# fakerlove1/HPFG

Hardware: AMD Instinct MI355X
Metric: labeled+unlabeled images/sec/node, U-Net 224x224 ACDC-shaped (Mean-Teacher step) (higher is better)
Workload: dtype bf16x3 (fp32 storage; products as split-bf16 MFMA hi*hi+hi*lo+lo*hi, fp32 accumulate); 1 GPU; mean_teacher_unet_224x224 (BASELINE configs[1]): U-Net 1ch->4cls, 8 labelled + 8 unlabelled per GPU, student fwd+bwd + train-mode teacher fwd + CE/Dice/MSE + SGD + EMA; size=224, hipgraph=True, sync_bn=False, parallelism=dp1, math=bf16x3

## Files before the change

hpfg_amd/_lib.py:

```python
from __future__ import annotations

import ctypes as C
import os
import threading

_HERE = os.path.dirname(os.path.abspath(__file__))
LIB_PATH = os.path.join(_HERE, "lib", "libhpfg_hip.so")

BN_MEAN, BN_RSTD, BN_SCALE, BN_SHIFT, BN_K1, BN_K2, BN_K3, BN_SPARE, BN_ROWS = range(9)
ACT_NONE, ACT_PLAIN, ACT_STRIDED, ACT_BNACT, ACT_BNACT_POOL, ACT_UP2X, ACT_DZ, ACT_SPLIT16, ACT_UPBWD = range(9)
OPT_CONV_THIN, OPT_FIRST_MFMA, OPT_FIRST_WGRAD, OPT_NARROW_DEEP, OPT_UPDATE_PACK = 0, 1, 2, 3, 4
LOSS_NSUM = 32
LOSS_MAX_CLASSES = 16
ACC_MAX_SHARDS = 8
VERSION = 141
RESIZE_TAPS = 36
SURFACE_SEGS = 32
MATH_F32, MATH_BF16X3 = 0, 1


class HipLibraryError(RuntimeError):
    pass


class Act(C.Structure):
    _fields_ = [("z", C.c_void_p), ("bn", C.c_void_p), ("aux", C.c_void_p), ("mode", C.c_int32), ("C", C.c_int32),
                ("Hs", C.c_int32), ("Ws", C.c_int32), ("pstride", C.c_int32), ("aux_pstride", C.c_int32),
                ("bn_stride", C.c_int32), ("bn_coff", C.c_int32), ("sn", C.c_int32), ("sc", C.c_int32), ("sy", C.c_int32),
                ("sx", C.c_int32), ("drop_p", C.c_float), ("drop_seed", C.c_uint32), ("drop_mask", C.c_void_p), ("seed_dev", C.c_void_p),
                ("bn_acc", C.c_void_p), ("bn_gamma", C.c_void_p), ("bn_beta", C.c_void_p), ("bn_count", C.c_float), ("bn_eps", C.c_float),
                ("bn_shards", C.c_int32), ("reserved1", C.c_int32)]


class ConvArgs(C.Structure):
    _fields_ = [("a0", Act), ("a1", Act), ("wpk", C.c_void_p), ("bias", C.c_void_p), ("out", C.c_void_p),
                ("stat_partials", C.c_void_p), ("out_pstride", C.c_int32), ("Cout", C.c_int32), ("CoutPad", C.c_int32),
                ("N", C.c_int32), ("H", C.c_int32), ("W", C.c_int32), ("taps", C.c_int32), ("math", C.c_int32),
                ("bwd_stats", C.c_int32), ("bwd_of", Act), ("out2", C.c_void_p), ("out_split", C.c_int32), ("out2_pstride", C.c_int32),
                ("stat_acc", C.c_void_p), ("stat_shards", C.c_int32), ("reserved2", C.c_int32), ("stage_out", C.c_void_p), ("side_sums", C.c_void_p)]


class WgradArgs(C.Structure):
    _fields_ = [("a0", Act), ("a1", Act), ("g", Act), ("slab", C.c_void_p), ("dw_oihw", C.c_void_p), ("Cin", C.c_int32),
                ("CinPad", C.c_int32), ("Cout", C.c_int32), ("CoutPad", C.c_int32), ("N", C.c_int32), ("H", C.c_int32),
                ("W", C.c_int32), ("taps", C.c_int32), ("S", C.c_int32), ("math", C.c_int32), ("defer_reduce", C.c_int32)]


class PeerX(C.Structure):
    _fields_ = [("mbox", C.c_void_p * 8), ("epoch", C.c_void_p), ("err", C.c_void_p), ("world", C.c_int32), ("rank", C.c_int32),
                ("slot", C.c_int32), ("cap", C.c_int32), ("slot_bytes", C.c_int64)]


class PeerBuf(C.Structure):
    _fields_ = [("win", C.c_void_p * 8), ("epoch", C.c_void_p), ("err", C.c_void_p), ("world", C.c_int32), ("rank", C.c_int32),
                ("slice", C.c_int64), ("n", C.c_int64), ("stride", C.c_int64)]


class FusedBwdArgs(C.Structure):
    _fields_ = [("d", ConvArgs), ("xa0", Act), ("xa1", Act), ("slab", C.c_void_p), ("Cin", C.c_int32), ("CinPad", C.c_int32),
                ("Cout", C.c_int32), ("CoutPad", C.c_int32)]


class AugSample(C.Structure):
    _fields_ = [("img_off", C.c_int64), ("lab_off", C.c_int64), ("h", C.c_int32), ("w", C.c_int32), ("mode", C.c_int32), ("k", C.c_int32),
# ... 162 lines not shown
    "hpfg_gelu_bwd": (_i, [_p, _p, _p, _l, _p]),
    "hpfg_patch_merge_fwd": (_i, [_p, _p, _i, _i, _i, _i, _p]),
    "hpfg_patch_merge_bwd": (_i, [_p, _p, _i, _i, _i, _i, _p]),
    "hpfg_attn_fwd_hd": (_i, [_p, _p, _p, _i, _i, _i, _i, _i, _f, _p]),
    "hpfg_attn_bwd_hd": (_i, [_p, _p, _p, _p, _p, _p, _i, _i, _i, _i, _i, _f, _p]),
    "hpfg_gemm_f32": (_i, [_p, _l, _l, _p, _l, _l, _p, _l, _i, _i, _i, _p, _i, _i, _p]),
    "hpfg_gemm_f32_splitk": (_i, [_p, _l, _l, _p, _l, _l, _p, _l, _i, _i, _i, _p, _i, _i, _p, _p]),
    "hpfg_gemm_f32_splits": (_i, [_i, _i, _i]),
    "hpfg_gemm_bf16x3": (_i, [_p, _l, _l, _p, _l, _l, _p, _l, _i, _i, _i, _p, _i, _i, _p]),
    "hpfg_gemm_bf16x3_splits": (_i, [_i, _i, _i]),
    "hpfg_gemm_bf16x3_splitk": (_i, [_p, _l, _l, _p, _l, _l, _p, _l, _i, _i, _i, _p, _i, _i, _p, _p]),
    "hpfg_gemm_bf16x3_ok": (_i, [_p, _l, _l, _p, _l, _l, _i, _i, _i]),
    "hpfg_gemm_tn_bf16x3": (_i, [_p, _p, _p, _p, _l, _i, _i, _i, _p]),
    "hpfg_gemm_tn_splits": (_i, [_l, _i, _i]),
    "hpfg_col_sum2": (_i, [_p, _l, _i, _l, _p, _p, _p]),
    "hpfg_col_sum_splits": (_i, [_l]),
    "hpfg_col_sum": (_i, [_p, _l, _i, _l, _p, _p]),
    "hpfg_relu_bwd": (_i, [_p, _p, _l, _p]),
    "hpfg_neck_pool_fwd": (_i, [_p, _i, _i, _i, _i, _i, _i, _p, _p, _p]),
    "hpfg_neck_pool_bwd": (_i, [_p, _p, _i, _i, _i, _i, _i, _p, _p]),
    "hpfg_l2norm_fwd": (_i, [_p, _i, _i, _i, _i, _i, _p, _p, _p]),
    "hpfg_l2norm_bwd": (_i, [_p, _p, _p, _i, _i, _i, _i, _i, _p, _p, _p]),
    "hpfg_ntxent_rows": (_i, [_p, _i, _f, _p, _p, _p]),
}

_lock = threading.Lock()
_lib = None


def load() -> C.CDLL:
    global _lib
    if _lib is not None:
        return _lib
    with _lock:
        if _lib is not None:
            return _lib
        if not os.path.exists(LIB_PATH):
            raise HipLibraryError(
                f"{LIB_PATH} not found: build it with `python -c 'import __graft_entry__ as g; g.build()'` "
                f"or `make -C hpfg_amd/csrc`. There is no CPU fallback for the HIP path.")
        lib = C.CDLL(LIB_PATH)
        for name, (res, args) in PROTOTYPES.items():
            fn = getattr(lib, name)
            fn.restype = res
            fn.argtypes = args
        if lib.hpfg_version() != VERSION:
            raise HipLibraryError(f"libhpfg_hip.so version {lib.hpfg_version()} != binding version {VERSION}; rebuild")
        if os.environ.get("HPFG_FIRST_WGRAD", "1") == "0":
            lib.hpfg_set_option(OPT_FIRST_WGRAD, 0)
        if os.environ.get("HPFG_NARROW_DEEP") is not None:
            lib.hpfg_set_option(OPT_NARROW_DEEP, int(os.environ["HPFG_NARROW_DEEP"]))
        if os.environ.get("HPFG_UPDATE_PACK", "1") == "0":
            lib.hpfg_set_option(OPT_UPDATE_PACK, 0)
        _lib = lib
    return _lib


def check(rc: int, what: str):
    if rc != 0:
        msg = load().hpfg_last_error().decode("utf-8", "replace")
        raise HipLibraryError(f"{what} failed (rc={rc}): {msg}")


def ptr(t):
    return None if t is None else t.data_ptr()


def none_act() -> Act:
    return Act()
```

hpfg_amd/csrc/conv_bf16_kernel.h:

```cpp
#pragma once
#include <stdlib.h>
#include "stage.h"

namespace hpfg_conv16 {

using namespace hpfg_stage;

template <int TH_, int TW_, int WM_, int WN_, int NI_, int TAPS_, int KC_>
struct Cfg {
  static constexpr int TH = TH_, TW = TW_, WM = WM_, WN = WN_, NI = NI_, TAPS = TAPS_, KC = KC_;
  static constexpr int MI = TH * TW / 16 / WM;
  static constexpr int BN = 16 * NI * WN;
  static constexpr int HALO = TAPS == 9 ? 1 : 0;
  static constexpr int HP = TH + 2 * HALO, WP = TW + 2 * HALO;
  static constexpr int RS = TW == 16 ? WP : (TAPS == 9 ? 24 : 8);
  static constexpr int NSLOT = (HP * RS + 15) / 16 * 16;
  static constexpr int NG = KC / 8;
  static constexpr int PLANE = NSLOT * 16;
  static constexpr int BUF_BYTES = NG * 2 * PLANE;
  static constexpr int KSTEPS = TAPS == 1 ? 1 : (KC == 32 ? 9 : 5);
  static constexpr int NPIECE = HP * WP * NG;
  static constexpr int NLD = (NPIECE + 255) / 256;
  static_assert(WM * WN == 4, "4 waves per workgroup");
  static_assert(256 % NG == 0, "a thread must keep one channel group");
  static_assert(KC == 32 || (KC == 16 && TAPS == 9), "two-tap K packing only for 3x3");
  static_assert(TAPS == 1 || NLD + 2 <= KSTEPS, "stage pipeline must fit into the k-steps of a chunk");
};

struct Piece {
  int ly, lx, lds, ok;
};
template <class C>
__device__ __forceinline__ Piece make_piece(int tid, int i) {
  Piece q;
  const int idx = tid + i * 256;
  const int pix = idx / C::NG, g = idx % C::NG;
  q.ok = idx < C::NPIECE;
  q.ly = pix / C::WP - C::HALO;
  q.lx = pix % C::WP - C::HALO;
  q.lds = (g * 2) * C::PLANE + ((pix / C::WP) * C::RS + pix % C::WP) * 16;
  return q;
}

template <class C, int KIND = HPFG_KIND_PLAIN, bool SIDE_ON = false>
__device__ __forceinline__ void store_piece(unsigned char* buf, const Piece& q, const f32x4& v0, const f32x4& v1, const HpfgConvArgs* p = nullptr,
                                            bool on = false, int n = 0, int gy = 0, int gx = 0, int c0 = 0, bool ok = false) {
  if (!q.ok) return;
  bf16x8 hi, lo;
  split_piece<KIND>(v0, v1, hi, lo);
  *reinterpret_cast<bf16x8*>(buf + q.lds) = hi;
  *reinterpret_cast<bf16x8*>(buf + q.lds + C::PLANE) = lo;
  if constexpr (SIDE_ON) {
    if (on && ok && q.ly >= 0 && q.ly < C::TH && q.lx >= 0 && q.lx < C::TW) {
      const int ct = p->a0.C + p->a1.C;
      __bf16* d = reinterpret_cast<__bf16*>(p->stage_out) + ((((long)n * p->H + gy) * p->W + gx) * ct + c0) * 2;
      *reinterpret_cast<bf16x8*>(d) = hi;
      *reinterpret_cast<bf16x8*>(d + 8) = lo;
    }
  }
}

template <class C>
__device__ __forceinline__ void load_b(bf16x8 (&bh)[C::NI], bf16x8 (&bl)[C::NI], const bf16x8* wpk, int ks, int ntn, int nt0, int lane) {
#pragma unroll
  for (int j = 0; j < C::NI; ++j) {
    const bf16x8* q = wpk + ((ks * ntn + nt0 + j) * 2) * 64 + lane;
    bh[j] = q[0];
    bl[j] = q[64];
  }
}

template <class C>
__device__ __forceinline__ void conv16_load_bias(const HpfgConvArgs& p, f32x4 (&bias)[C::NI], int lane, int nt0) {
#pragma unroll
// ... 135 lines not shown
      }
      s1[j][r] = a;
      s2[j][r] = b;
    }
  if ((lane & 15) == 0) {
#pragma unroll
    for (int j = 0; j < C::NI; ++j) {
      const int cl = (wn * C::NI + j) * 16 + (lane >> 4) * 4;
      *reinterpret_cast<f32x4*>(ldsf + (0 * C::WM + wm) * C::BN + cl) = s1[j];
      *reinterpret_cast<f32x4*>(ldsf + (1 * C::WM + wm) * C::BN + cl) = s2[j];
    }
  }
  __syncthreads();
  if (tid < 2 * C::BN) {
    const int which = tid / C::BN, cl = tid % C::BN;
    float t = 0.f;
#pragma unroll
    for (int w = 0; w < C::WM; ++w) t += ldsf[(which * C::WM + w) * C::BN + cl];
    const int co = cb * C::BN + cl;
    if (BWD && p.bwd_stats && which == 1 && co < p.Cout) {
      float sg = 0.f;
#pragma unroll
      for (int w = 0; w < C::WM; ++w) sg += ldsf[w * C::BN + cl];
      const float* tb = p.bwd_of.bn + p.bwd_of.bn_coff + co;
      t = tb[HPFG_BN_RSTD * p.bwd_of.bn_stride] * (t - tb[HPFG_BN_MEAN * p.bwd_of.bn_stride] * sg);
    }
    if (p.stat_acc && co < p.Cout)
      hpfg_acc_add(p.stat_acc, p.CoutPad, ((int)blockIdx.z * (int)gridDim.y + (int)blockIdx.y) * (int)gridDim.x + (int)blockIdx.x & (p.stat_shards - 1), which, co, t);
    if (p.stat_partials && co < p.CoutPad) p.stat_partials[((long)row * 2 + which) * p.CoutPad + co] = t;
  }
}

#define HPFG16_MFMA3(ACC, AH, AL, BH, BL)                              \
  ACC = __builtin_amdgcn_mfma_f32_16x16x32_bf16(BH, AH, ACC, 0, 0, 0); \
  ACC = __builtin_amdgcn_mfma_f32_16x16x32_bf16(BL, AH, ACC, 0, 0, 0); \
  ACC = __builtin_amdgcn_mfma_f32_16x16x32_bf16(BH, AL, ACC, 0, 0, 0);

template <class C>
struct UpGeo {
  using P = UpPatch<C::TH, C::TW>;
  static constexpr int SW = P::SW;
  static constexpr int NPIECE = P::SH * P::SW * C::NG;
  static constexpr int BYTES = P::SH * P::SW * C::KC * 4;
  static_assert(NPIECE <= 256, "one source piece per thread");
};
template <int KIND>
constexpr int eff_nr() { return KIND == HPFG_KIND_CAT ? 2 : RawCount<KIND>::N; }

template <class C, int KIND>
constexpr int wg_per_cu() {
  return (C::KSTEPS == 5 && C::NI == 1 && RawCount<KIND>::N <= 2) ? 3 : 2;
}

template <class C, int KIND, int BWD = 0>
__global__ __launch_bounds__(256, (wg_per_cu<C, KIND>())) void conv_bf16x3_kernel(HpfgConvArgs p, int tiles_x, int tiles_y) {
  static_assert(C::TAPS == 9, "persistent kernel is the 3x3 path");
  constexpr int STAT_BYTES = 2 * 4 * C::BN * 4;
  constexpr int NR = eff_nr<KIND>();
  constexpr bool CATK = KIND == HPFG_KIND_CAT;
  constexpr int UP_BYTES = CATK ? UpGeo<C>::BYTES : 0;
  __shared__ __attribute__((aligned(16))) unsigned char lds[2 * C::BUF_BYTES + STAT_BYTES + UP_BYTES];
  float* ldsf = reinterpret_cast<float*>(lds + 2 * C::BUF_BYTES);
  float* ldsU = reinterpret_cast<float*>(lds + 2 * C::BUF_BYTES + STAT_BYTES);
  (void)ldsU;
  constexpr bool TABK = tab_in_lds<KIND>();
  __shared__ __attribute__((aligned(16))) float ldsBN[TABK ? tab_rows<KIND>() * HPFG_BN_CMAX : 4];
  (void)ldsBN;
  const int tid = threadIdx.x, lane = tid & 63, wave = tid >> 6;
  const int wm = wave % C::WM, wn = wave / C::WM;
  const int cb = blockIdx.y;
  const int H = p.H, W = p.W;
  const int ntiles = tiles_x * tiles_y, nwork = ntiles * p.N;
  const ActCtx cx0 = make_ctx(p.a0);
  constexpr bool SIDE = KIND != HPFG_KIND_PLAIN && C::TH == 4;
  const bool dzw = SIDE && p.stage_out != nullptr && cb == 0;
  (void)dzw;
#ifdef HPFG_TRACE
  const bool tr_on = (p.math & 0x2000) && tid == 0;
  unsigned long long* tr_buf = reinterpret_cast<unsigned long long*>(p.stat_partials) + 256 * ((long)blockIdx.y * gridDim.x + blockIdx.x);
  int tr_i = 0;
#endif
  HPFG_TR_REAL(11)
  HPFG_TR(1)

  f32x4 acc[C::MI][C::NI];
#pragma unroll
  for (int m = 0; m < C::MI; ++m)
#pragma unroll
    for (int j = 0; j < C::NI; ++j) acc[m][j] = f32x4{0.f, 0.f, 0.f, 0.f};

  const int kg = lane >> 4;
  const int gl = C::KC == 32 ? kg : (kg & 1);
  int aoff[C::MI];
#pragma unroll
  for (int m = 0; m < C::MI; ++m) {
    const int pxl = (wm * C::MI + m) * 16 + (lane & 15);
    aoff[m] = (gl * 2) * C::PLANE + ((pxl / C::TW) * C::RS + (pxl % C::TW)) * 16;
  }
  int toff[C::KSTEPS];
#pragma unroll
  for (int s = 0; s < C::KSTEPS; ++s) {
    int tap = C::KC == 32 ? s : 2 * s + (kg >> 1);
    tap = tap > 8 ? 8 : tap;
    toff[s] = ((tap / 3) * C::RS + (tap % 3)) * 16;
  }
  Piece pc[C::NLD];
#pragma unroll
  for (int i = 0; i < C::NLD; ++i) pc[i] = make_piece<C>(tid, i);
  const int g8 = (tid % C::NG) * 8;

  const int cin_total = p.a0.C + p.a1.C;
  const int nchunks = (cin_total + C::KC - 1) / C::KC;
  const int ntn = p.CoutPad / 16;
  const int nt0 = (cb * C::WN + wn) * C::NI;
  const bf16x8* wpk = reinterpret_cast<const bf16x8*>(p.wpk);

  const TileWalk tw = tile_walk(nwork, gridDim.x >= 8 ? 8 : 1);
  const int wend = tw.wend, G = tw.step;
  int w = tw.w;
  if (w >= wend) {
    if (p.stat_partials && threadIdx.x < 2 * C::BN) {
      const int co = cb * C::BN + (int)threadIdx.x % C::BN;
      if (co < p.CoutPad) p.stat_partials[((long)blockIdx.x * 2 + (int)threadIdx.x / C::BN) * p.CoutPad + co] = 0.f;
    }
    return;
  }
  int n = w / ntiles, tyi = (w % ntiles) / tiles_x, txi = (w % ntiles) % tiles_x;
  int ty0 = tyi * C::TH, tx0 = txi * C::TW;
  const int gn = G / ntiles, gty = (G % ntiles) / tiles_x, gtx = (G % ntiles) % tiles_x;
  f32x4 s1[C::NI], s2[C::NI];
#pragma unroll
  for (int j = 0; j < C::NI; ++j) {
    s1[j] = f32x4{0.f, 0.f, 0.f, 0.f};
    s2[j] = s1[j];
  }
  constexpr bool TIGHT = C::TAPS == 9 && C::KSTEPS == 5 && C::NI >= 2 && eff_nr<KIND>() >= 4;
  f32x4 bias[C::NI];
  if (!TIGHT) conv16_load_bias<C>(p, bias, lane, nt0);
  Tab tab;
  HPFG_TR(2)
  {
    const int c0 = g8;
    const bool chv = c0 < cin_total;
    const int c0c = chv ? c0 : 0;
    RawPiece<KIND> raw0[C::NLD];
#pragma unroll
    for (int i = 0; i < C::NLD; ++i) {
      const int gy = ty0 + pc[i].ly, gx = tx0 + pc[i].lx;
      const bool ok = pc[i].ok && chv && gy >= 0 && gy < H && gx >= 0 && gx < W;
      issue_piece<KIND>(raw0[i], p.a0, p.a1, cx0, n, clampi(gy, 0, H - 1), clampi(gx, 0, W - 1), c0c, ok);
    }
    if constexpr (TABK) {
      fill_tables_lds<KIND>(p.a0, ldsBN, p.a0.C, tid, 256);
      __syncthreads();
      load_tables_lds<KIND>(tab, ldsBN, p.a0, c0c);
    } else {
      load_tables<KIND>(tab, p.a0, c0, chv);
    }
#pragma unroll
    for (int i = 0; i < C::NLD; ++i) {
      const int gy = ty0 + pc[i].ly, gx = tx0 + pc[i].lx;
      const bool ok = pc[i].ok && chv && gy >= 0 && gy < H && gx >= 0 && gx < W;
      f32x4 v0, v1;
      const int gyc = clampi(gy, 0, H - 1), gxc = clampi(gx, 0, W - 1);
      finish_piece<KIND>(v0, v1, raw0[i], tab, p.a0, p.a1, cx0, n, gyc, gxc, c0c, ok);
      store_piece<C, KIND, SIDE>(lds, pc[i], v0, v1, &p, dzw, n, gyc, gxc, c0c, ok);
    }
  }
  constexpr int BR = C::KSTEPS == 5 ? 5 : (C::NI == 1 ? 9 : 3), BD = BR - 1;
  static_assert(C::KSTEPS % BR == 0, "ring size must divide the k-steps of a chunk");
  const int kperiod = nchunks * C::KSTEPS;
  bf16x8 bh[BR][C::NI], bl[BR][C::NI];
#pragma unroll
  for (int d = 0; d < BD; ++d) load_b<C>(bh[d], bl[d], wpk, d % kperiod, ntn, nt0, lane);
  HPFG_TR(3)
  __syncthreads();
  HPFG_TR(4)
  int item = 0;
  while (true) {
    for (int ch = 0; ch < nchunks; ++ch, ++item) {
      const unsigned char* cur = lds + (item & 1) * C::BUF_BYTES;
      unsigned char* nxt = lds + ((item + 1) & 1) * C::BUF_BYTES;
      const bool last_chunk = ch + 1 == nchunks;
      const int w2 = w + G;
      const bool more = !last_chunk || w2 < wend;
      const int nch = last_chunk ? 0 : ch + 1;
      int nn = n, nty = ty0, ntx = tx0;
      if (last_chunk && more) {
        int x2 = txi + gtx, y2 = tyi + gty;
        nn = n + gn;
        if (x2 >= tiles_x) {
          x2 -= tiles_x;
          ++y2;
        }
        if (y2 >= tiles_y) {
          y2 -= tiles_y;
          ++nn;
        }
        nty = y2 * C::TH;
        ntx = x2 * C::TW;
      }
      const int c0n = nch * C::KC + g8;
      const bool chvn = more && c0n < cin_total && !(p.math & 0x400);
      const int c0c = c0n < cin_total ? c0n : 0;
      if constexpr (TABK) load_tables_lds<KIND>(tab, ldsBN, p.a0, c0c);
      else if (!TIGHT || (more && nchunks > 1)) load_tables<KIND>(tab, p.a0, c0c, true);
      constexpr bool DEEP = (NR <= 2 || C::NLD <= 2) && (C::KC != 32 || CATK);
      constexpr int SK = CATK ? HPFG_KIND_BNACT : KIND;
      RawPiece<SK> raw[DEEP ? C::NLD : 2];
      const bool up_next = CATK && nch * C::KC >= p.a0.C;
      f32x4 rawU[2];
      int sy_base = 0, sx_base = 0;
      if (CATK && up_next) {
        sy_base = up_base(nty - 1, p.a1.Hs);
        sx_base = up_base(ntx - 1, p.a1.Ws);
        const int cu = (c0n < cin_total ? c0n : p.a0.C) - p.a0.C;
        up_patch_issue<UpGeo<C>::SW>(rawU, p.a1, nn, sy_base, sx_base, tid / C::NG, cu);
      } else if (DEEP) {
#pragma unroll
        for (int i = 0; i < C::NLD; ++i) {
          const int gy = nty + pc[i].ly, gx = ntx + pc[i].lx;
          const bool ok = pc[i].ok && chvn && gy >= 0 && gy < H && gx >= 0 && gx < W;
          issue_piece<SK>(raw[DEEP ? i : 0], p.a0, p.a1, cx0, nn, clampi(gy, 0, H - 1), clampi(gx, 0, W - 1), c0c, ok);
        }
      }
      HPFG_TR(5)
      constexpr int Q = C::KSTEPS * C::MI;
      constexpr int AD0 = wg_per_cu<C, KIND>() == 3 ? 2 : (C::NI == 1 ? 4 : (TIGHT ? 0 : 2));
      constexpr int AD = AD0 < Q ? AD0 : Q;
      constexpr int AR = AD + 1;
      constexpr bool FENCE = !TIGHT;
      bf16x8 ah[AR], al[AR];
#pragma unroll
      for (int q = 0; q < AD; ++q) {
        ah[q % AR] = *reinterpret_cast<const bf16x8*>(cur + aoff[q % C::MI] + toff[q / C::MI]);
        al[q % AR] = *reinterpret_cast<const bf16x8*>(cur + aoff[q % C::MI] + toff[q / C::MI] + C::PLANE);
      }
      if (FENCE) __builtin_amdgcn_sched_barrier(0x216);
#pragma unroll
      for (int q = 0; q < Q; ++q) {
        const int s = q / C::MI, m = q % C::MI;
        if (q + AD < Q) {
          const int q2 = q + AD;
          ah[q2 % AR] = *reinterpret_cast<const bf16x8*>(cur + aoff[q2 % C::MI] + toff[q2 / C::MI]);
          al[q2 % AR] = *reinterpret_cast<const bf16x8*>(cur + aoff[q2 % C::MI] + toff[q2 / C::MI] + C::PLANE);
        }
        if (m == 0) {
          if (!DEEP) {
            if (s >= 2 && s - 2 < C::NLD) {
              const int i = s - 2 < C::NLD ? s - 2 : 0;
              const int gy = nty + pc[i].ly, gx = ntx + pc[i].lx;
              const bool ok = pc[i].ok && chvn && gy >= 0 && gy < H && gx >= 0 && gx < W;
              f32x4 v0, v1;
              finish_piece<SK>(v0, v1, raw[i & 1], tab, p.a0, p.a1, cx0, nn, clampi(gy, 0, H - 1), clampi(gx, 0, W - 1), c0c, ok);
              store_piece<C, SK, SIDE>(nxt, pc[i], v0, v1, &p, dzw, nn, gy, gx, c0c, ok);
            }
            if (s < C::NLD) {
              const int i = s < C::NLD ? s : 0;
              const int gy = nty + pc[i].ly, gx = ntx + pc[i].lx;
              const bool ok = pc[i].ok && chvn && gy >= 0 && gy < H && gx >= 0 && gx < W;
              issue_piece<SK>(raw[i & 1], p.a0, p.a1, cx0, nn, clampi(gy, 0, H - 1), clampi(gx, 0, W - 1), c0c, ok);
            }
          }
          int ksn = ch * C::KSTEPS + s + BD;
          ksn = ksn >= kperiod ? ksn - kperiod : ksn;
          load_b<C>(bh[(s + BD) % BR], bl[(s + BD) % BR], wpk, ksn, ntn, nt0, lane);
        }
#pragma unroll
        for (int j = 0; j < C::NI; ++j) { HPFG16_MFMA3(acc[m][j], ah[q % AR], al[q % AR], bh[s % BR][j], bl[s % BR][j]) }
        if (FENCE) __builtin_amdgcn_sched_barrier(0x216);
      }
      HPFG_TR(6)
      if (CATK && up_next) {
        using UG = UpGeo<C>;
        if (tid < UG::NPIECE) up_patch_park<C::KC>(ldsU, rawU, tid / C::NG, g8);
        __syncthreads();
#pragma unroll
        for (int i = 0; i < C::NLD; ++i) {
          const int gy = nty + pc[i].ly, gx = ntx + pc[i].lx;
          const bool ok = pc[i].ok && chvn && gy >= 0 && gy < H && gx >= 0 && gx < W;
          f32x4 v0, v1;
          up_blend<C::KC, UG::SW>(v0, v1, ldsU, p.a1, clampi(gy, 0, H - 1), clampi(gx, 0, W - 1), sy_base, sx_base, g8, ok);
          store_piece<C, HPFG_KIND_PLAIN, SIDE>(nxt, pc[i], v0, v1, &p, dzw, nn, gy, gx, c0c, ok);
        }
      } else if (DEEP) {
#pragma unroll
        for (int i = 0; i < C::NLD; ++i) {
          const int gy = nty + pc[i].ly, gx = ntx + pc[i].lx;
          const bool ok = pc[i].ok && chvn && gy >= 0 && gy < H && gx >= 0 && gx < W;
          f32x4 v0, v1;
          finish_piece<SK>(v0, v1, raw[DEEP ? i : 0], tab, p.a0, p.a1, cx0, nn, clampi(gy, 0, H - 1), clampi(gx, 0, W - 1), c0c, ok);
          store_piece<C, SK, SIDE>(nxt, pc[i], v0, v1, &p, dzw, nn, gy, gx, c0c, ok);
        }
      }
      HPFG_TR(7)
      __syncthreads();
      HPFG_TR(8)
    }
    conv16_store_tile<C, BWD>(p, acc, s1, s2, bias, lane, wm, nt0, n, ty0, tx0, TIGHT);
    HPFG_TR(9)
#pragma unroll
    for (int m = 0; m < C::MI; ++m)
#pragma unroll
      for (int j = 0; j < C::NI; ++j) acc[m][j] = f32x4{0.f, 0.f, 0.f, 0.f};
    w += G;
    if (w >= wend) break;
    txi += gtx;
    tyi += gty;
    n += gn;
    if (txi >= tiles_x) {
      txi -= tiles_x;
      ++tyi;
    }
    if (tyi >= tiles_y) {
      tyi -= tiles_y;
      ++n;
    }
    ty0 = tyi * C::TH;
    tx0 = txi * C::TW;
  }
  conv16_flush_stats<C, BWD>(p, s1, s2, ldsf, tid, lane, wm, wn, cb, (int)blockIdx.x);
  HPFG_TR(10)
  HPFG_TR_REAL(12)
}

template <class C, int KIND, int BWD = 0>
__global__ __launch_bounds__(256) void conv1x1_bf16x3_kernel(HpfgConvArgs p, int tiles_x, int tiles_y) {
  static_assert(C::TAPS == 1, "1x1 path");
  constexpr int STAT_BYTES = 2 * 4 * C::BN * 4;
  constexpr int NR = RawCount<KIND>::N;
  __shared__ __attribute__((aligned(16))) unsigned char lds[C::BUF_BYTES + STAT_BYTES];
  float* ldsf = reinterpret_cast<float*>(lds + C::BUF_BYTES);
  constexpr bool TABK = tab_in_lds<KIND>();
  __shared__ __attribute__((aligned(16))) float ldsBN[TABK ? tab_rows<KIND>() * HPFG_BN_CMAX : 4];
  (void)ldsBN;
  constexpr bool UPB = KIND == HPFG_KIND_UPB;
  __shared__ short upI[UPB ? C::TH + C::TW : 1][HPFG_UPB_TAPS];
  __shared__ float upW[UPB ? C::TH + C::TW : 1][HPFG_UPB_TAPS];
  __shared__ __attribute__((aligned(16))) float upS[UPB ? 256 * 8 : 4];
  (void)upI;
  (void)upW;
  (void)upS;
  const int tid = threadIdx.x, lane = tid & 63, wave = tid >> 6;
  const int wm = wave % C::WM, wn = wave / C::WM;
  const int tile = blockIdx.x, n = blockIdx.y, cb = blockIdx.z;
  const int ty0 = (tile / tiles_x) * C::TH, tx0 = (tile % tiles_x) * C::TW;
  const int H = p.H, W = p.W;
  const ActCtx cx0 = make_ctx(p.a0);
  f32x4 acc[C::MI][C::NI];
#pragma unroll
  for (int m = 0; m < C::MI; ++m)
#pragma unroll
// ... 91 lines not shown
      }
      if (side && p.side_sums) {
        *reinterpret_cast<f32x4*>(upS + tid * 8) = cs0;
        *reinterpret_cast<f32x4*>(upS + tid * 8 + 4) = cs1;
      }
    } else {
#pragma unroll
    for (int i = 0; i < C::NLD; ++i) {
      const Piece q = make_piece<C>(tid, i);
      const int gy = ty0 + q.ly, gx = tx0 + q.lx;
      const bool ok = q.ok && chv && gy < H && gx < W;
      RawPiece<KIND> raw;
      f32x4 v0, v1;
      const int gyc = clampi(gy, 0, H - 1), gxc = clampi(gx, 0, W - 1), c0c = chv ? c0 : 0;
      issue_piece<KIND>(raw, p.a0, p.a1, cx0, n, gyc, gxc, c0c, ok);
      finish_piece<KIND>(v0, v1, raw, tab, p.a0, p.a1, cx0, n, gyc, gxc, c0c, ok);
      store_piece<C, KIND>(lds, q, v0, v1);
    }
    }
    bf16x8 bh[C::NI], bl[C::NI];
    load_b<C>(bh, bl, wpk, ch, ntn, nt0, lane);
    __syncthreads();
    if constexpr (UPB) {
      if (side && p.side_sums && tid < C::KC) {
        const int g = tid >> 3, j = tid & 7;
        float tsum = 0.f;
        for (int k = g; k < 256; k += C::NG) tsum += upS[k * 8 + j];
        const int cch = ch * C::KC + tid;
        if (cch < p.a0.C) p.side_sums[(long)wg_row * p.a0.C + cch] = tsum;
      }
    }
#pragma unroll
    for (int m = 0; m < C::MI; ++m) {
      const bf16x8 ah = *reinterpret_cast<const bf16x8*>(lds + aoff[m]);
      const bf16x8 al = *reinterpret_cast<const bf16x8*>(lds + aoff[m] + C::PLANE);
#pragma unroll
      for (int j = 0; j < C::NI; ++j) { HPFG16_MFMA3(acc[m][j], ah, al, bh[j], bl[j]) }
    }
  }
  f32x4 s1[C::NI], s2[C::NI];
#pragma unroll
  for (int j = 0; j < C::NI; ++j) {
    s1[j] = f32x4{0.f, 0.f, 0.f, 0.f};
    s2[j] = s1[j];
  }
  f32x4 bias[C::NI];
  conv16_load_bias<C>(p, bias, lane, nt0);
  conv16_store_tile<C, BWD>(p, acc, s1, s2, bias, lane, wm, nt0, n, ty0, tx0);
  __syncthreads();
  conv16_flush_stats<C, BWD>(p, s1, s2, ldsf, tid, lane, wm, wn, cb, n * (tiles_x * tiles_y) + tile);
}

template <class C, int KIND>
int persistent_grid(const HpfgConvArgs& a) {
  const int tx = (a.W + C::TW - 1) / C::TW, ty = (a.H + C::TH - 1) / C::TH;
  const int lds_bytes = 2 * C::BUF_BYTES + 2 * 4 * C::BN * 4;
  int per_cu = 160 * 1024 / lds_bytes;
  const int reg_cap = wg_per_cu<C, KIND>();
  if (per_cu > reg_cap) per_cu = reg_cap;
  if (per_cu < 1) per_cu = 1;
  const long nwork = (long)tx * ty * a.N;
  const long gy = a.CoutPad / C::BN;
  long cap = 256L * per_cu / (gy > 0 ? gy : 1);
  if (cap < 1) cap = 1;
  const long rounds = (nwork + cap - 1) / cap;
  return (int)((nwork + rounds - 1) / rounds);
}

template <class C, int KIND>
int launch_cfg(const HpfgConvArgs& a, hipStream_t st, int* rows_only) {
  int tx = (a.W + C::TW - 1) / C::TW, ty = (a.H + C::TH - 1) / C::TH;
  if (rows_only) {
    if constexpr (C::TAPS == 9) *rows_only = persistent_grid<C, KIND>(a);
    else *rows_only = tx * ty * a.N;
    return 0;
  }
  if constexpr (C::TAPS == 9) {
    dim3 grid((unsigned)persistent_grid<C, KIND>(a), a.CoutPad / C::BN);
    if (a.stat_acc) HPFG_ACC_CHECK((long)grid.x * grid.y, a.stat_shards, "conv_fwd");
    if constexpr (KIND == HPFG_KIND_DZ || KIND == HPFG_KIND_PLAIN) {
      if constexpr (C::TH == 4) {
        if (a.bwd_stats == 2) {
          hipLaunchKernelGGL((conv_bf16x3_kernel<C, KIND, 2>), grid, dim3(256), 0, st, a, tx, ty);
          return hpfg_launch_status("conv_bf16x3_kernel<bwd stats + pool>");
        }
      }
      if (a.bwd_stats == 2) {
        hpfg_set_error("conv_fwd: bwd_stats == 2 is built for H or W not a multiple of 16");
        return -1;
      }
      if (a.bwd_stats) {
        hipLaunchKernelGGL((conv_bf16x3_kernel<C, KIND, 1>), grid, dim3(256), 0, st, a, tx, ty);
        return hpfg_launch_status("conv_bf16x3_kernel<bwd stats>");
      }
    }
    hipLaunchKernelGGL((conv_bf16x3_kernel<C, KIND>), grid, dim3(256), 0, st, a, tx, ty);
  } else {
    dim3 grid(tx * ty, a.N, a.CoutPad / C::BN);
    if (a.stat_acc) HPFG_ACC_CHECK((long)grid.x * grid.y * grid.z, a.stat_shards, "conv_fwd(1x1)");
    if constexpr (KIND == HPFG_KIND_DZ || KIND == HPFG_KIND_PLAIN || KIND == HPFG_KIND_UPB) {
      if (a.bwd_stats) {
        hipLaunchKernelGGL((conv1x1_bf16x3_kernel<C, KIND, 1>), grid, dim3(256), 0, st, a, tx, ty);
        return hpfg_launch_status("conv1x1_bf16x3_kernel<bwd stats>");
      }
    }
    hipLaunchKernelGGL((conv1x1_bf16x3_kernel<C, KIND>), grid, dim3(256), 0, st, a, tx, ty);
  }
  return hpfg_launch_status("conv_bf16x3_kernel");
}

template <int KIND, int TAPS>
int conv_dispatch_kind(const HpfgConvArgs& a, hipStream_t st, int* rows_only) {
  const bool big = (a.H % 16 == 0) && (a.W % 16 == 0);
  const int cp = a.CoutPad;
  constexpr int KCB = TAPS == 9 ? 16 : 32;
  if (big) {
    if constexpr (TAPS == 1) {
      if (cp % 64 == 0) return launch_cfg<Cfg<16, 16, 4, 1, 4, TAPS, KCB>, KIND>(a, st, rows_only);
    }
    if (cp % 32 == 0) return launch_cfg<Cfg<16, 16, 4, 1, 2, TAPS, KCB>, KIND>(a, st, rows_only);
    return launch_cfg<Cfg<16, 16, 4, 1, 1, TAPS, KCB>, KIND>(a, st, rows_only);
  }
  if constexpr (TAPS == 9) {
    {
      const long tiles = (long)a.N * ((a.H + 3) / 4) * ((a.W + 15) / 16);
      if (cp % 64 == 0 && tiles * (cp / 64) <= hpfg_opt(HPFG_OPT_NARROW_DEEP))
        return launch_cfg<Cfg<4, 16, 2, 2, 1, TAPS, 32>, KIND>(a, st, rows_only);
    }
    if (cp % 64 == 0) return launch_cfg<Cfg<4, 16, 1, 4, 1, TAPS, 32>, KIND>(a, st, rows_only);
    if (cp % 32 == 0) return launch_cfg<Cfg<4, 16, 2, 2, 1, TAPS, 32>, KIND>(a, st, rows_only);
    return launch_cfg<Cfg<4, 16, 4, 1, 1, TAPS, 32>, KIND>(a, st, rows_only);
  }
  const long nwork = (long)a.N * ((a.H + 7) / 8) * ((a.W + 7) / 8);
  if (cp % 128 == 0 && nwork * (cp / 128) >= 512) return launch_cfg<Cfg<8, 8, 1, 4, 2, TAPS, 32>, KIND>(a, st, rows_only);
  if (cp % 64 == 0 && (nwork * (cp / 64) >= 512 || cp % 32 != 0)) return launch_cfg<Cfg<8, 8, 1, 4, 1, TAPS, 32>, KIND>(a, st, rows_only);
  if (cp % 32 == 0) return launch_cfg<Cfg<8, 8, 2, 2, 1, TAPS, 32>, KIND>(a, st, rows_only);
  return launch_cfg<Cfg<8, 8, 4, 1, 1, TAPS, 32>, KIND>(a, st, rows_only);
}

}

constexpr int HPFG_THIN_NONE = -100;
int hpfg_conv_thin_try(const HpfgConvArgs& a, hipStream_t st, int* rows_only);
int hpfg_conv16_launch_plain(const HpfgConvArgs& a, hipStream_t st, int* rows_only);
int hpfg_conv16_launch_bnact(const HpfgConvArgs& a, hipStream_t st, int* rows_only);
int hpfg_conv16_launch_pool(const HpfgConvArgs& a, hipStream_t st, int* rows_only);
int hpfg_conv16_launch_cat(const HpfgConvArgs& a, hipStream_t st, int* rows_only);
int hpfg_conv16_launch_dz(const HpfgConvArgs& a, hipStream_t st, int* rows_only);
int hpfg_conv16_launch_upb(const HpfgConvArgs& a, hipStream_t st, int* rows_only);
// ... 1 lines not shown
```

hpfg_amd/csrc/misc.hip:

```cpp
#include <stdarg.h>
#include <string.h>
#include "stage.h"

static thread_local char g_err[512] = "";
extern "C" void hpfg_set_error(const char* fmt, ...) {
  va_list ap;
  va_start(ap, fmt);
  vsnprintf(g_err, sizeof(g_err), fmt, ap);
  va_end(ap);
}
extern "C" const char* hpfg_last_error(void) { return g_err; }
extern "C" int hpfg_version(void) { return HPFG_VERSION; }

static int g_opt[HPFG_OPT_COUNT] = {1, 1, 1, 128, 1};
int hpfg_opt(int which) { return which >= 0 && which < HPFG_OPT_COUNT ? g_opt[which] : 0; }
extern "C" int hpfg_get_option(int which) { return hpfg_opt(which); }
extern "C" int hpfg_set_option(int which, int value) {
  HPFG_ARG_CHECK(which >= 0 && which < HPFG_OPT_COUNT, "set_option: unknown option %d", which);
  const int old = g_opt[which];
  g_opt[which] = value;
  return old;
}

namespace {

__global__ __launch_bounds__(256) void pack_weights_kernel(const HpfgPackDesc* __restrict__ table, long long* __restrict__ counters, int n_counters,
                                                           int* __restrict__ seed_word, int seed_add, long long* __restrict__ zero, long n_zero) {
  if (blockIdx.x == 0 && blockIdx.y == 0) {
    for (int i = threadIdx.x; i < n_counters; i += 256) counters[i] += 1;
    if (threadIdx.x == 0 && seed_word && seed_add) *seed_word = (*seed_word + seed_add) & 0x7FFFFFFF;
  }
  for (long i = ((long)blockIdx.y * gridDim.x + blockIdx.x) * 256 + threadIdx.x; i < n_zero; i += (long)gridDim.x * gridDim.y * 256) zero[i] = 0;
  const HpfgPackDesc d = table[blockIdx.y];
  const long total = (long)d.taps * d.CinPad * d.CoutPad;
  const int nt_f = d.CoutPad / 16, nch_f = d.CinPad / 16;
  const int nt_d = d.CinPad / 16, nch_d = d.CoutPad / 16;
  for (long i = blockIdx.x * 256L + threadIdx.x; i < total; i += (long)gridDim.x * 256) {
    int ks = (int)(i & 3), lane = (int)((i >> 2) & 63);
    long r = i >> 8;
    if (d.wpk_fwd) {
      int nt = (int)(r % nt_f), ch = (int)((r / nt_f) % nch_f), tap = (int)(r / ((long)nt_f * nch_f));
      int co = nt * 16 + (lane & 15), ci = ch * 16 + ks * 4 + (lane >> 4);
      d.wpk_fwd[i] = (co < d.Cout && ci < d.Cin) ? d.w_oihw[((long)co * d.Cin + ci) * d.taps + tap] : 0.f;
    }
    if (d.wpk_dgrad) {
      int nt = (int)(r % nt_d), ch = (int)((r / nt_d) % nch_d), tap = (int)(r / ((long)nt_d * nch_d));
      int co = ch * 16 + ks * 4 + (lane >> 4), ci = nt * 16 + (lane & 15);
      d.wpk_dgrad[i] = (co < d.Cout && ci < d.Cin) ? d.w_oihw[((long)co * d.Cin + ci) * d.taps + (d.taps - 1 - tap)] : 0.f;
    }
    if (i < d.CoutPad) d.bias_pad[i] = (i < d.Cout && d.b) ? d.b[i] : 0.f;
  }
  const int ksteps = d.taps == 1 ? 1 : (d.kc == 32 ? 9 : 5);
  for (int dir = 0; dir < 2; ++dir) {
    __bf16* out = reinterpret_cast<__bf16*>(dir == 0 ? d.wpk16_fwd : d.wpk16_dgrad);
    if (!out) continue;
    const int Kch = dir == 0 ? d.Cin : d.Cout;
    const int ntn = (dir == 0 ? d.CoutPad : d.CinPad) / 16;
    const int nchunks = (Kch + d.kc - 1) / d.kc;
    const long tot = (long)nchunks * ksteps * ntn * 512;
    for (long i = blockIdx.x * 256L + threadIdx.x; i < tot; i += (long)gridDim.x * 256) {
      const int j = (int)(i & 7), lane = (int)((i >> 3) & 63);
      const long r = i >> 9;
      const int nt = (int)(r % ntn), ks = (int)(r / ntn);
      const int chunk = ks / ksteps, s = ks % ksteps;
      const int kl = 8 * (lane >> 4) + j;
      int tap, kch;
      if (d.taps == 1) { tap = 0; kch = chunk * 32 + kl; }
// ... 574 lines not shown
```

include/hpfg_hip.h:

```cpp
#ifndef HPFG_HIP_H
#define HPFG_HIP_H

#include <stdint.h>

#ifdef __cplusplus
extern "C" {
#endif

#define HPFG_VERSION 141
enum { HPFG_MATH_F32 = 0, HPFG_MATH_BF16X3 = 1 };

enum { HPFG_BN_MEAN = 0, HPFG_BN_RSTD = 1, HPFG_BN_SCALE = 2, HPFG_BN_SHIFT = 3,
       HPFG_BN_K1 = 4, HPFG_BN_K2 = 5, HPFG_BN_K3 = 6, HPFG_BN_SPARE = 7, HPFG_BN_ROWS = 8 };

enum {
  HPFG_ACT_NONE = 0,
  HPFG_ACT_PLAIN = 1,
  HPFG_ACT_STRIDED = 2,
  HPFG_ACT_BNACT = 3,
  HPFG_ACT_BNACT_POOL = 4,
  HPFG_ACT_UP2X = 5,
  HPFG_ACT_DZ = 6,
  HPFG_ACT_SPLIT16 = 7,
  HPFG_ACT_UPBWD = 8
// ... 37 lines not shown
  int32_t bwd_stats;
  HpfgAct bwd_of;
  float* out2;
  int32_t out_split;
  int32_t out2_pstride;
  long long* stat_acc;
  int32_t stat_shards;
  int32_t reserved2;
  float* stage_out;
  float* side_sums;
} HpfgConvArgs;
#define HPFG_ACC_MAX_SHARDS 8
#define HPFG_ACC_WORDS(C, shards) ((shards) * 2 * 2 * (C))

typedef struct HpfgWgradArgs {
  HpfgAct a0, a1;
  HpfgAct g;
  float* slab;
  float* dw_oihw;
  int32_t Cin, CinPad, Cout, CoutPad;
  int32_t N, H, W, taps;
  int32_t S;
  int32_t math;
  int32_t defer_reduce;
} HpfgWgradArgs;

typedef struct HpfgFusedBwdArgs {
  HpfgConvArgs d;
  HpfgAct xa0, xa1;
  float* slab;
  int32_t Cin, CinPad, Cout, CoutPad;
} HpfgFusedBwdArgs;

typedef struct HpfgSlabDesc {
  const float* slab;
  float* dw_oihw;
  int32_t S, taps, Cin, CinPad, Cout, CoutPad;
} HpfgSlabDesc;

typedef struct HpfgPackDesc {
  const float* w_oihw;
  const float* b;
  float* wpk_fwd;
  float* wpk_dgrad;
  float* bias_pad;
  void* wpk16_fwd;
  void* wpk16_dgrad;
  int32_t Cout, Cin, CoutPad, CinPad, taps;
  int32_t kc;
} HpfgPackDesc;

int hpfg_version(void);
const char* hpfg_last_error(void);
enum { HPFG_OPT_CONV_THIN = 0, HPFG_OPT_FIRST_MFMA = 1, HPFG_OPT_FIRST_WGRAD = 2, HPFG_OPT_NARROW_DEEP = 3, HPFG_OPT_UPDATE_PACK = 4, HPFG_OPT_COUNT = 5 };
int hpfg_get_option(int which);
int hpfg_set_option(int which, int value);

int hpfg_conv3x3_first_fwd(const HpfgAct* x, const float* w_oihw, const float* bias, float* out, float* stat_partials,
                           int N, int H, int W, int Cin, int Cout, void* stream);
int hpfg_conv_first_rows(int N, int H, int W);
int hpfg_conv3x3_first_fwd_acc(const HpfgAct* x, const float* w_oihw, const float* bias, float* out, float* stat_partials, long long* stat_acc,
                               int stat_shards, int N, int H, int W, int Cin, int Cout, void* stream);
int hpfg_conv_fwd(const HpfgConvArgs* args, void* stream);
int hpfg_conv_stat_blocks(int N, int H, int W);
int hpfg_conv_stat_rows(const HpfgConvArgs* args);
int hpfg_bn_fwd_finalize(const float* partials, int nblk, const double* sums, double count, const float* gamma, const float* beta,
                         float* running_mean, float* running_var, float momentum, float eps, float* bn, int C, void* stream);
typedef struct HpfgBnAccDesc {
  const long long* acc;
  const float* gamma;
  const float* beta;
  float* running_mean;
  float* running_var;
  float* bn;
  int32_t C;
  float count;
  int32_t shards;
  int32_t reserved;
} HpfgBnAccDesc;
int hpfg_bn_acc_finalize(const HpfgBnAccDesc* table_dev, const HpfgBnAccDesc* table_host, int nlayers, float momentum, float eps, void* stream);
typedef struct HpfgBnAccBwdDesc {
  long long* acc;
  const float* gamma;
  float* bn;
  float* dgamma;
  float* dbeta;
  int32_t C;
  float count;
  int32_t shards;
  int32_t reserved;
} HpfgBnAccBwdDesc;
int hpfg_bn_acc_bwd_finalize(const HpfgBnAccBwdDesc* table_dev, const HpfgBnAccBwdDesc* table_host, int nlayers, void* stream);
int hpfg_bn_bwd_reduce_acc(const HpfgAct* g, int N, int H, int W, long long* acc, int shards, void* stream);
int hpfg_bn_bwd_reduce_pool_acc(const HpfgAct* g, const float* dP, int dp_pstride, int N, int Hp, int Wp, long long* acc, int shards, void* stream);
int hpfg_reduce_partials(const float* partials, int nblk, int C, double* sums, void* stream);
int hpfg_bn_eval_table(const float* gamma, const float* beta, const float* running_mean, const float* running_var, float eps,
                       float* bn, int C, void* stream);
int hpfg_conv3x3_first_fwd_bump(const HpfgAct* x, const float* w_oihw, const float* bias, float* out, float* stat_partials, long long* stat_acc,
                                int stat_shards, long long* counters, int n_counters, int32_t* seed_word, int seed_add, int N, int H, int W, int Cin,
                                int Cout, void* stream);
int hpfg_conv_kc(int H, int W, int taps);
long hpfg_wpk16_elems(int Kchannels, int NchannelsPad, int taps, int kc);
int hpfg_pack_weights(const HpfgPackDesc* table_dev, const HpfgPackDesc* table_host, int nlayers, void* stream);
int hpfg_pack_weights_bump(const HpfgPackDesc* table_dev, const HpfgPackDesc* table_host, int nlayers, long long* counters, int n_counters,
                           int32_t* seed_word, int seed_add, long long* zero_words, long n_zero, void* stream);
int hpfg_act_materialize(const HpfgAct* a0, const HpfgAct* a1, int N, int H, int W, float* out, void* stream);
int hpfg_dropout_mask(uint8_t* out, long n_elems, float p, uint32_t seed, const uint32_t* seed_dev, void* stream);
// ... 233 lines not shown
```

Baseline: 7818 images/s.

## Park BN stat accumulators in LDS and add optional 3-per-CU lean conv variant

For the 3x3 bf16x3 persistent conv configs with 4-row tiles and 32-channel chunks, the per-thread BN statistic accumulators now live in LDS between tiles, and the bias is reloaded at store time instead of held in registers. The aim is to cut register pressure. An opt-in variant (HPFG_CONV_PER_CU=3) serializes the halo-piece loads, shrinks the B-fragment ring and targets three workgroups per CU. The LDS parking and bias reload also run by default, which costs extra LDS traffic and footprint, and that larger footprint enters the grid sizing computation.

```diff
diff --git a/hpfg_amd/_lib.py b/hpfg_amd/_lib.py
--- a/hpfg_amd/_lib.py
+++ b/hpfg_amd/_lib.py
@@ -9,7 +9,7 @@
 
 BN_MEAN, BN_RSTD, BN_SCALE, BN_SHIFT, BN_K1, BN_K2, BN_K3, BN_SPARE, BN_ROWS = range(9)
 ACT_NONE, ACT_PLAIN, ACT_STRIDED, ACT_BNACT, ACT_BNACT_POOL, ACT_UP2X, ACT_DZ, ACT_SPLIT16, ACT_UPBWD = range(9)
-OPT_CONV_THIN, OPT_FIRST_MFMA, OPT_FIRST_WGRAD, OPT_NARROW_DEEP, OPT_UPDATE_PACK = 0, 1, 2, 3, 4
+OPT_CONV_THIN, OPT_FIRST_MFMA, OPT_FIRST_WGRAD, OPT_NARROW_DEEP, OPT_UPDATE_PACK, OPT_CONV_PER_CU = 0, 1, 2, 3, 4, 5
 LOSS_NSUM = 32
 LOSS_MAX_CLASSES = 16
 ACC_MAX_SHARDS = 8
@@ -278,6 +278,8 @@
             lib.hpfg_set_option(OPT_NARROW_DEEP, int(os.environ["HPFG_NARROW_DEEP"]))
         if os.environ.get("HPFG_UPDATE_PACK", "1") == "0":
             lib.hpfg_set_option(OPT_UPDATE_PACK, 0)
+        if os.environ.get("HPFG_CONV_PER_CU") is not None:
+            lib.hpfg_set_option(OPT_CONV_PER_CU, int(os.environ["HPFG_CONV_PER_CU"]))
         _lib = lib
     return _lib
 
diff --git a/hpfg_amd/csrc/conv_bf16_kernel.h b/hpfg_amd/csrc/conv_bf16_kernel.h
--- a/hpfg_amd/csrc/conv_bf16_kernel.h
+++ b/hpfg_amd/csrc/conv_bf16_kernel.h
@@ -20,6 +20,7 @@
   static constexpr int BUF_BYTES = NG * 2 * PLANE;
   static constexpr int KSTEPS = TAPS == 1 ? 1 : (KC == 32 ? 9 : 5);
   static constexpr int NPIECE = HP * WP * NG;
+  static constexpr bool LEAN = TH == 4 && KC == 32 && TAPS == 9;
   static constexpr int NLD = (NPIECE + 255) / 256;
   static_assert(WM * WN == 4, "4 waves per workgroup");
   static_assert(256 % NG == 0, "a thread must keep one channel group");
@@ -261,8 +262,8 @@
   return (C::KSTEPS == 5 && C::NI == 1 && RawCount<KIND>::N <= 2) ? 3 : 2;
 }
 
-template <class C, int KIND, int BWD = 0>
-__global__ __launch_bounds__(256, (wg_per_cu<C, KIND>())) void conv_bf16x3_kernel(HpfgConvArgs p, int tiles_x, int tiles_y) {
+template <class C, int KIND, int BWD = 0, int PER_CU = wg_per_cu<C, KIND>()>
+__global__ __launch_bounds__(256, PER_CU) void conv_bf16x3_kernel(HpfgConvArgs p, int tiles_x, int tiles_y) {
   static_assert(C::TAPS == 9, "persistent kernel is the 3x3 path");
   constexpr int STAT_BYTES = 2 * 4 * C::BN * 4;
   constexpr int NR = eff_nr<KIND>();
@@ -275,6 +276,10 @@
   constexpr bool TABK = tab_in_lds<KIND>();
   __shared__ __attribute__((aligned(16))) float ldsBN[TABK ? tab_rows<KIND>() * HPFG_BN_CMAX : 4];
   (void)ldsBN;
+  constexpr bool LEAN = C::LEAN && PER_CU == 3;
+  constexpr bool PARK = C::LEAN;
+  __shared__ f32x4 ldsS[PARK ? 2 * C::NI * 256 : 1];
+  (void)ldsS;
   const int tid = threadIdx.x, lane = tid & 63, wave = tid >> 6;
   const int wm = wave % C::WM, wn = wave / C::WM;
   const int cb = blockIdx.y;
@@ -342,10 +347,15 @@
   for (int j = 0; j < C::NI; ++j) {
     s1[j] = f32x4{0.f, 0.f, 0.f, 0.f};
     s2[j] = s1[j];
+    if constexpr (PARK) {
+      ldsS[j * 256 + tid] = s1[j];
+      ldsS[(C::NI + j) * 256 + tid] = s2[j];
+    }
   }
   constexpr bool TIGHT = C::TAPS == 9 && C::KSTEPS == 5 && C::NI >= 2 && eff_nr<KIND>() >= 4;
+  constexpr bool RELOAD = TIGHT || C::LEAN;
   f32x4 bias[C::NI];
-  if (!TIGHT) conv16_load_bias<C>(p, bias, lane, nt0);
+  if (!RELOAD) conv16_load_bias<C>(p, bias, lane, nt0);
   Tab tab;
   HPFG_TR(2)
   {
@@ -376,7 +386,7 @@
       store_piece<C, KIND, SIDE>(lds, pc[i], v0, v1, &p, dzw, n, gyc, gxc, c0c, ok);
     }
   }
-  constexpr int BR = C::KSTEPS == 5 ? 5 : (C::NI == 1 ? 9 : 3), BD = BR - 1;
+  constexpr int BR = C::KSTEPS == 5 ? 5 : (C::NI == 1 && !LEAN ? 9 : 3), BD = BR - 1;
   static_assert(C::KSTEPS % BR == 0, "ring size must divide the k-steps of a chunk");
   const int kperiod = nchunks * C::KSTEPS;
   bf16x8 bh[BR][C::NI], bl[BR][C::NI];
@@ -412,11 +422,14 @@
       const int c0n = nch * C::KC + g8;
       const bool chvn = more && c0n < cin_total && !(p.math & 0x400);
       const int c0c = c0n < cin_total ? c0n : 0;
-      if constexpr (TABK) load_tables_lds<KIND>(tab, ldsBN, p.a0, c0c);
+      if constexpr (TABK && LEAN) {
+      } else if constexpr (TABK) load_tables_lds<KIND>(tab, ldsBN, p.a0, c0c);
       else if (!TIGHT || (more && nchunks > 1)) load_tables<KIND>(tab, p.a0, c0c, true);
       constexpr bool DEEP = (NR <= 2 || C::NLD <= 2) && (C::KC != 32 || CATK);
       constexpr int SK = CATK ? HPFG_KIND_BNACT : KIND;
-      RawPiece<SK> raw[DEEP ? C::NLD : 2];
+      constexpr bool SER = LEAN && !DEEP;
+      static_assert(!SER || 3 * C::NLD <= C::KSTEPS, "the pieces of a chunk, one after the other, must fit into its k-steps");
+      RawPiece<SK> raw[DEEP ? C::NLD : (SER ? 1 : 2)];
       const bool up_next = CATK && nch * C::KC >= p.a0.C;
       f32x4 rawU[2];
       int sy_base = 0, sx_base = 0;
@@ -435,7 +448,7 @@
       }
       HPFG_TR(5)
       constexpr int Q = C::KSTEPS * C::MI;
-      constexpr int AD0 = wg_per_cu<C, KIND>() == 3 ? 2 : (C::NI == 1 ? 4 : (TIGHT ? 0 : 2));
+      constexpr int AD0 = PER_CU == 3 ? 2 : (C::NI == 1 ? 4 : (TIGHT ? 0 : 2));
       constexpr int AD = AD0 < Q ? AD0 : Q;
       constexpr int AR = AD + 1;
       constexpr bool FENCE = !TIGHT;
@@ -456,19 +469,20 @@
         }
         if (m == 0) {
           if (!DEEP) {
-            if (s >= 2 && s - 2 < C::NLD) {
-              const int i = s - 2 < C::NLD ? s - 2 : 0;
+            if (SER ? (s % 3 == 2 && s / 3 < C::NLD) : (s >= 2 && s - 2 < C::NLD)) {
+              const int i = SER ? (s / 3 < C::NLD ? s / 3 : 0) : (s - 2 < C::NLD ? s - 2 : 0);
               const int gy = nty + pc[i].ly, gx = ntx + pc[i].lx;
               const bool ok = pc[i].ok && chvn && gy >= 0 && gy < H && gx >= 0 && gx < W;
               f32x4 v0, v1;
-              finish_piece<SK>(v0, v1, raw[i & 1], tab, p.a0, p.a1, cx0, nn, clampi(gy, 0, H - 1), clampi(gx, 0, W - 1), c0c, ok);
+              if constexpr (TABK && LEAN) load_tables_lds<KIND>(tab, ldsBN, p.a0, c0c);
+              finish_piece<SK>(v0, v1, raw[SER ? 0 : (i & 1)], tab, p.a0, p.a1, cx0, nn, clampi(gy, 0, H - 1), clampi(gx, 0, W - 1), c0c, ok);
               store_piece<C, SK, SIDE>(nxt, pc[i], v0, v1, &p, dzw, nn, gy, gx, c0c, ok);
             }
-            if (s < C::NLD) {
-              const int i = s < C::NLD ? s : 0;
+            if (SER ? (s % 3 == 0 && s / 3 < C::NLD) : s < C::NLD) {
+              const int i = SER ? (s / 3 < C::NLD ? s / 3 : 0) : (s < C::NLD ? s : 0);
               const int gy = nty + pc[i].ly, gx = ntx + pc[i].lx;
               const bool ok = pc[i].ok && chvn && gy >= 0 && gy < H && gx >= 0 && gx < W;
-              issue_piece<SK>(raw[i & 1], p.a0, p.a1, cx0, nn, clampi(gy, 0, H - 1), clampi(gx, 0, W - 1), c0c, ok);
+              issue_piece<SK>(raw[SER ? 0 : (i & 1)], p.a0, p.a1, cx0, nn, clampi(gy, 0, H - 1), clampi(gx, 0, W - 1), c0c, ok);
             }
           }
           int ksn = ch * C::KSTEPS + s + BD;
@@ -493,6 +507,7 @@
           store_piece<C, HPFG_KIND_PLAIN, SIDE>(nxt, pc[i], v0, v1, &p, dzw, nn, gy, gx, c0c, ok);
         }
       } else if (DEEP) {
+        if constexpr (TABK && LEAN) load_tables_lds<KIND>(tab, ldsBN, p.a0, c0c);
 #pragma unroll
         for (int i = 0; i < C::NLD; ++i) {
           const int gy = nty + pc[i].ly, gx = ntx + pc[i].lx;
@@ -506,7 +521,21 @@
       __syncthreads();
       HPFG_TR(8)
     }
-    conv16_store_tile<C, BWD>(p, acc, s1, s2, bias, lane, wm, nt0, n, ty0, tx0, TIGHT);
+    if constexpr (PARK) {
+#pragma unroll
+      for (int j = 0; j < C::NI; ++j) {
+        s1[j] = ldsS[j * 256 + tid];
+        s2[j] = ldsS[(C::NI + j) * 256 + tid];
+      }
+    }
+    conv16_store_tile<C, BWD>(p, acc, s1, s2, bias, lane, wm, nt0, n, ty0, tx0, RELOAD);
+    if constexpr (PARK) {
+#pragma unroll
+      for (int j = 0; j < C::NI; ++j) {
+        ldsS[j * 256 + tid] = s1[j];
+        ldsS[(C::NI + j) * 256 + tid] = s2[j];
+      }
+    }
     HPFG_TR(9)
 #pragma unroll
     for (int m = 0; m < C::MI; ++m)
@@ -704,11 +733,28 @@
 }
 
 template <class C, int KIND>
+int conv_per_cu() {
+  return (C::LEAN && hpfg_opt(HPFG_OPT_CONV_PER_CU) == 3) ? 3 : wg_per_cu<C, KIND>();
+}
+template <class C, int KIND, int BWD>
+void launch_persistent(dim3 grid, hipStream_t st, const HpfgConvArgs& a, int tx, int ty) {
+  if constexpr (C::LEAN) {
+    if (conv_per_cu<C, KIND>() == 3) {
+      hipLaunchKernelGGL((conv_bf16x3_kernel<C, KIND, BWD, 3>), grid, dim3(256), 0, st, a, tx, ty);
+      return;
+    }
+  }
+  hipLaunchKernelGGL((conv_bf16x3_kernel<C, KIND, BWD>), grid, dim3(256), 0, st, a, tx, ty);
+}
+
+template <class C, int KIND>
 int persistent_grid(const HpfgConvArgs& a) {
   const int tx = (a.W + C::TW - 1) / C::TW, ty = (a.H + C::TH - 1) / C::TH;
-  const int lds_bytes = 2 * C::BUF_BYTES + 2 * 4 * C::BN * 4;
+  int lds_bytes = 2 * C::BUF_BYTES + 2 * 4 * C::BN * 4;
+  if (C::LEAN)
+    lds_bytes += 2 * C::NI * 256 * 16 + (tab_in_lds<KIND>() ? tab_rows<KIND>() * HPFG_BN_CMAX * 4 : 0) + (KIND == HPFG_KIND_CAT ? UpGeo<C>::BYTES : 0);
   int per_cu = 160 * 1024 / lds_bytes;
-  const int reg_cap = wg_per_cu<C, KIND>();
+  const int reg_cap = (C::LEAN && a.stat_partials) ? 2 : conv_per_cu<C, KIND>();
   if (per_cu > reg_cap) per_cu = reg_cap;
   if (per_cu < 1) per_cu = 1;
   const long nwork = (long)tx * ty * a.N;
@@ -733,7 +779,7 @@
     if constexpr (KIND == HPFG_KIND_DZ || KIND == HPFG_KIND_PLAIN) {
       if constexpr (C::TH == 4) {
         if (a.bwd_stats == 2) {
-          hipLaunchKernelGGL((conv_bf16x3_kernel<C, KIND, 2>), grid, dim3(256), 0, st, a, tx, ty);
+          launch_persistent<C, KIND, 2>(grid, st, a, tx, ty);
           return hpfg_launch_status("conv_bf16x3_kernel<bwd stats + pool>");
         }
       }
@@ -742,11 +788,11 @@
         return -1;
       }
       if (a.bwd_stats) {
-        hipLaunchKernelGGL((conv_bf16x3_kernel<C, KIND, 1>), grid, dim3(256), 0, st, a, tx, ty);
+        launch_persistent<C, KIND, 1>(grid, st, a, tx, ty);
         return hpfg_launch_status("conv_bf16x3_kernel<bwd stats>");
       }
     }
-    hipLaunchKernelGGL((conv_bf16x3_kernel<C, KIND>), grid, dim3(256), 0, st, a, tx, ty);
+    launch_persistent<C, KIND, 0>(grid, st, a, tx, ty);
   } else {
     dim3 grid(tx * ty, a.N, a.CoutPad / C::BN);
     if (a.stat_acc) HPFG_ACC_CHECK((long)grid.x * grid.y * grid.z, a.stat_shards, "conv_fwd(1x1)");
diff --git a/hpfg_amd/csrc/misc.hip b/hpfg_amd/csrc/misc.hip
--- a/hpfg_amd/csrc/misc.hip
+++ b/hpfg_amd/csrc/misc.hip
@@ -12,7 +12,7 @@
 extern "C" const char* hpfg_last_error(void) { return g_err; }
 extern "C" int hpfg_version(void) { return HPFG_VERSION; }
 
-static int g_opt[HPFG_OPT_COUNT] = {1, 1, 1, 128, 1};
+static int g_opt[HPFG_OPT_COUNT] = {1, 1, 1, 128, 1, 2};
 int hpfg_opt(int which) { return which >= 0 && which < HPFG_OPT_COUNT ? g_opt[which] : 0; }
 extern "C" int hpfg_get_option(int which) { return hpfg_opt(which); }
 extern "C" int hpfg_set_option(int which, int value) {
diff --git a/include/hpfg_hip.h b/include/hpfg_hip.h
--- a/include/hpfg_hip.h
+++ b/include/hpfg_hip.h
@@ -113,7 +113,8 @@
 
 int hpfg_version(void);
 const char* hpfg_last_error(void);
-enum { HPFG_OPT_CONV_THIN = 0, HPFG_OPT_FIRST_MFMA = 1, HPFG_OPT_FIRST_WGRAD = 2, HPFG_OPT_NARROW_DEEP = 3, HPFG_OPT_UPDATE_PACK = 4, HPFG_OPT_COUNT = 5 };
+enum { HPFG_OPT_CONV_THIN = 0, HPFG_OPT_FIRST_MFMA = 1, HPFG_OPT_FIRST_WGRAD = 2, HPFG_OPT_NARROW_DEEP = 3, HPFG_OPT_UPDATE_PACK = 4, HPFG_OPT_CONV_PER_CU = 5,
+       HPFG_OPT_COUNT = 6 };
 int hpfg_get_option(int which);
 int hpfg_set_option(int which, int value);
 
```

After: 7831 images/s (median of 6 runs). Within noise of the previous version (+0.2%).
